# franciscotln/cosmology-model-fit

Hardware: AMD Instinct MI355X
Metric: walker-logL evals/s, Pantheon+ 1701-SN full-cov chi2, theta resident in HBM (higher is better)
Workload: dtype f64; 1 GPU; Pantheon+-shaped 1701-SN full-cov flat-LCDM chi2 + prior, 4096 walkers per GPU per step (BASELINE configs[1] at N=1), G=4000, theta resident in HBM; workload_key=pantheon, walkers_per_gpu=4096, walkers_total=4096, n_sn=1701, n_grid=4000, ndim=4, parallelism=walkers sharded over 1 GPU(s)

## Files before the change

### cosmology-model-fit_amd/_lib.py

```python
from __future__ import annotations

import ctypes as C
import os
import subprocess

_HERE = os.path.dirname(os.path.abspath(__file__))
LIB_PATH = os.environ.get("COSMOFIT_LIB") or os.path.join(_HERE, "libcosmofit_hip.so")
CSRC = os.path.join(_HERE, "csrc")

CF_ABI_VERSION = 11
CF_P_NSLOTS = 15
SLOTS = ("offset", "H0", "Om", "obh2", "och2", "w0", "wa", "v", "rd", "fcc", "lin", "v2", "v3", "s8", "fs8err")

CF_EZ_LATE_FLAT, CF_EZ_PHYSICAL = 0, 1
CF_FDE_LCDM, CF_FDE_WCDM, CF_FDE_THAWING, CF_FDE_CPL = 0, 1, 2, 3
CF_OUT_CHI2, CF_OUT_LOGL, CF_OUT_LOGP = 0, 1, 2
CF_SOLVE_BLOCKED_TRSM, CF_SOLVE_INVERSE_GEMM, CF_SOLVE_AUTO = 0, 1, 2
SOLVE_MODES = {"blocked": CF_SOLVE_BLOCKED_TRSM, "inverse": CF_SOLVE_INVERSE_GEMM, "auto": CF_SOLVE_AUTO}
CF_CMB_NONE = 0
STATUS = {0: "CF_OK", -1: "CF_ERR_INVALID", -2: "CF_ERR_NO_DEVICE", -3: "CF_ERR_HIP", -4: "CF_ERR_NOT_POSDEF",
          -5: "CF_ERR_UNSUPPORTED", -6: "CF_ERR_ILL_CONDITIONED"}


class CosmofitError(RuntimeError):
# ... 200 lines not shown
    "cf_last_kernel_ms": (C.c_int, [_VP, C.POINTER(C.c_float * 2)]),
    "cf_enable_timing": (C.c_int, [_VP, C.c_int]),
    "cf_set_timing_stride": (C.c_int, [_VP, C.c_int]),
    "cf_timed_calls": (C.c_int64, [_VP]),
    "cf_kernel_ms": (C.c_int, [_VP, _I64, C.POINTER(C.c_float * 2)]),
    "cf_kernel_ms3": (C.c_int, [_VP, _I64, C.POINTER(C.c_float * 3)]),
    "cf_walker_form": (C.c_int, [_VP, _I64]),
    "cf_interp_hermite": (C.c_int, [_VP, _I64, _VP, _VP, _VP, _I64, _VP]),
    "cf_interp_pchip": (C.c_int, [_VP, _I64, _VP, _VP, _I64, _VP]),
    "cf_solve_triangular": (C.c_int, [_VP, _I64, _I64, _VP, _I64, _VP]),
    "cf_selftest_invpack_host": (C.c_int, [_VP, _I64, _I64, _VP, C.POINTER(C.c_double), C.POINTER(C.c_double)]),
    "cf_selftest_log10": (C.c_int, [_VP, _I64, _VP]),
    "cf_selftest_log10_tab": (C.c_int, [_VP, _I64, _VP]),
    "cf_selftest_exp_tab": (C.c_int, [_VP, _I64, _VP]),
    "cf_selftest_pos_ops": (C.c_int, [_VP, _VP, _I64, _VP]),
    "cf_ens_active_count": (_I64, [C.c_uint64, _I32, _I32, _I64, _I64]),
    "cf_ens_comp_count": (_I64, [C.c_uint64, _I32, _I32, _I64]),
    "cf_ens_active_set": (C.c_int, [C.c_uint64, _I32, _I32, _I64, _I64, _VP, _VP, _VP]),
    "cf_ens_kde_prepare": (C.c_int, [_VP, _I64, _I32, _I32, _I32, C.c_uint64, _VP, _VP, _VP]),
    "cf_ens_propose": (C.c_int, [_I32, _VP, _I64, _I32, _I32, _I32, C.c_uint64, _VP, _I64, C.c_uint64, C.c_double,
                                 C.c_double, _VP, _VP, _VP, _VP, _VP]),
    "cf_ens_accept": (C.c_int, [_VP, _VP, _I64, C.c_int32, C.c_uint64, _VP, _VP, _VP, _VP, _VP, _VP, _VP]),
    "cf_ens_accept_record": (C.c_int, [_VP, _VP, _I64, C.c_int32, C.c_uint64, _VP, _VP, _VP, _VP, _VP, _VP, _VP, _VP, _VP,
                                       _VP]),
    "cf_chain_mean": (C.c_int, [_VP, _I64, _I64, _VP, _VP]),
    "cf_chain_lagsum": (C.c_int, [_VP, _VP, _I64, _I64, _I64, _I32, _VP, _VP]),
    "cf_chain_acf_mean": (C.c_int, [_VP, _VP, _I64, _I32, _I32, _VP, _VP]),
    "cf_marg_bin": (C.c_int, [_VP, _I64, _I32, _VP, _I32, _VP, _VP]),
    "cf_marg_hist": (C.c_int, [_VP, _VP, C.c_double, _I64, _I32, _I32, _VP, _I32, _VP, _VP, _I32, _VP]),
    "cf_kde_sum_device": (C.c_int, [_VP, _VP, _I64, _I32, _VP, _I64, _I64, _VP, _VP, _VP]),
# ... 98 lines not shown
```

### cosmology-model-fit_amd/csrc/cf_stream_pack.h

```cpp
#ifndef CF_STREAM_PACK_H
#define CF_STREAM_PACK_H

#include <algorithm>
#include <cmath>
#include <cstdint>
#include <numeric>
#include <vector>

#include "cosmofit_device.h"

struct cf_stream_plan {
  std::vector<int32_t> row;
  int32_t seg_off[CF_STREAM_MAX_SEGS + 1];
  int32_t n_seg;
  double max_step, zp1_max;
};

static inline bool cf_stream_assign(const double* z_cmb, const double* step, int64_t n_sn, int n_grid, double inv_step, double z_max,
                                    cf_stream_plan& plan) {
  if (n_grid < 2 || n_grid > CF_STREAM_SEG * CF_STREAM_MAX_SEGS || n_sn < 0 || n_sn > INT32_MAX - CF_STREAM_REC_SLACK) return false;
  plan.n_seg = (n_grid + CF_STREAM_SEG - 1) / CF_STREAM_SEG;
  std::vector<int32_t> node((size_t)n_sn);
  plan.max_step = 0.0;
  plan.zp1_max = 1.0;
// ... 5 lines not shown
  }
  plan.row.resize((size_t)n_sn);
  std::iota(plan.row.begin(), plan.row.end(), 0);
  std::stable_sort(plan.row.begin(), plan.row.end(), [&](int32_t a, int32_t b) { return node[(size_t)a] < node[(size_t)b]; });
  for (int s = 0; s <= CF_STREAM_MAX_SEGS; ++s) plan.seg_off[s] = (int32_t)n_sn;
  int s = 0;
  plan.seg_off[0] = 0;
  for (int64_t j = 0; j < n_sn; ++j) {
    const int sj = cf_stream_segment(node[(size_t)plan.row[(size_t)j]], plan.n_seg);
    while (s < sj) plan.seg_off[++s] = (int32_t)j;
  }
  while (s < CF_STREAM_MAX_SEGS) plan.seg_off[++s] = (int32_t)n_sn;
  return true;
}

#endif
```

### cosmology-model-fit_amd/csrc/cf_wave_scan.h

```cpp
#ifndef CF_WAVE_SCAN_H
#define CF_WAVE_SCAN_H

#include <hip/hip_runtime.h>

template <int CTRL, int ROW_MASK>
__device__ __forceinline__ double dpp_move(double v) {
  const int lo = __builtin_amdgcn_update_dpp(0, __double2loint(v), CTRL, ROW_MASK, 0xF, false);
  const int hi = __builtin_amdgcn_update_dpp(0, __double2hiint(v), CTRL, ROW_MASK, 0xF, false);
  return __hiloint2double(hi, lo);
}

__device__ __forceinline__ double wave_inclusive_scan(double v) {
  v += dpp_move<0x111, 0xF>(v);
  v += dpp_move<0x112, 0xF>(v);
  v += dpp_move<0x114, 0xF>(v);
  v += dpp_move<0x118, 0xF>(v);
  v += dpp_move<0x142, 0xA>(v);
  v += dpp_move<0x143, 0xC>(v);
  return v;
}

#endif
```

### cosmology-model-fit_amd/csrc/cosmofit_api.hip

```cpp
#include <hip/hip_runtime.h>
#include <sys/prctl.h>

#include <cmath>
#include <cstdio>
#include <cstdlib>
#include <chrono>
#include <cstring>
#include <algorithm>
#include <atomic>
#include <utility>
#include <condition_variable>
#include <memory>
#include <mutex>
#include <string>
#include <thread>
#include <vector>

#include "../../include/cosmofit.h"
#include "cf_pack.h"
#include "cf_stream_pack.h"
#include "cosmofit_device.h"
#include "cosmofit_infl.h"
#include "cosmofit_mock.h"
#include "cosmofit_resid.h"
// ... 154 lines not shown
CF_DECLARE_TRIGEMM_SMALL(8, false, 2)
#define CF_DECLARE_TRIGEMM(NP, PF)                                                                                                       \
  extern template __global__ void tri_gemm_chi2_kernel<NP, PF>(const cf_epilogue*, const d2*, int, int, int, const double*, int64_t,     \
                                                               const double*, int64_t, double*, unsigned int*, const double*, double*,  \
                                                               int, unsigned long long*, double*, int, int, int, int, int,              \
                                                               unsigned long long*, unsigned long long);
CF_DECLARE_TRIGEMM(1, 2)
CF_DECLARE_TRIGEMM(2, 2)
extern "C" __global__ void finalize_kernel(cf_epilogue d, const double* theta, int64_t W, const double* chi2_extra,
                                           double* out, int out_kind, unsigned long long* nonfinite, unsigned long long* done_flag,
                                           unsigned long long done_seq);
extern "C" __global__ void interp_kernel(const double* xq, int64_t nq, const double* x, const double* y,
                                         const double* yp, int64_t n, double* out, int mode);
extern "C" __global__ void log10_selftest_kernel(const double* x, int64_t n, double* out, int mode, const cf_d2* tab);
extern "C" __global__ void pos_ops_selftest_kernel(const double* a, const double* b, int64_t n, double* out);
extern "C" __global__ void pad_rhs_kernel(const double* b, int64_t nrhs, int64_t n, int64_t n_ld, double* delta);

static thread_local std::string g_err;

static void default_shape(int& ks, int& tc) {
  ks = 2;
  tc = 4;
}
#define CF_PROBE_LIMIT 1e-11

static int pack_default(const double* L, int64_t n, int64_t ld, cf_host_pack& hp, double* probe_rel = nullptr) {
  int ks, tc;
  default_shape(ks, tc);
  int rc = cf_pack_cholesky(L, n, ld, hp, ks, tc);
  if (rc == 0 && probe_rel) *probe_rel = cf_pack_probe(hp, L, ld);
// ... 127 lines not shown
  InversePack ipack;
  DevBuf partial, arrivals;
  DevBuf partial4;
  DevBuf epi;
  cf_epilogue epi_host{};
  hipStream_t stream = nullptr;
  hipStream_t last_stream = nullptr;
  bool has_last = false;
  std::vector<hipEvent_t> ev;
  int timing_slots = 0, timing_stride = 1;
  int64_t timed_calls = 0, eval_calls = 0;
  cf_dev_desc d{};
  PackedFactor pack;
  DevBuf z_cmb, z_hel, obs, sn_step, sn_rec, log10_tab;
  DevBuf stream_rec, stream_row;
  cf_stream_args sargs{};
  DevBuf bao_z, bao_val, bao_inv_cov, bao_qty, gl_x, gl_w, fixed_mu, cc_z, cc_h, cc_inv_cov, nu_grid, ln_grid, nu_sw, ln_sw, exp2_tab, sn_lin, sn_dir;
  DevBuf theta, out, delta, ypk, chi2_extra, nonfinite;
  DevBuf fs8_z, fs8_val, fs8_inv_cov, fs8_fid, fs8_step_of, fs8_order, fs8_tab, fs8_pts;
  DevBuf bao_nodes, bao_base;
  PinnedBuf done_flags;
  unsigned long long done_seq = 0;
  int done_armed = 0;
  bool theta_on_host = false;
  bool has_small_blocks = false;
  bool has_growth = false;
  cf_qsr_state* qsr = nullptr;
  int64_t max_walkers = 0;
  double pack_probe_rel = 0.0;
  int cu_count = 0;
// ... 410 lines not shown
        rec[i] = cf_d4{d.has_vstep ? 1.0 + c->sn_z_cmb[i] : c->sn_z_cmb[i], d.lin_in_rec ? c->sn_lin_coef[i] : step[i],
                       1.0 + c->sn_z_hel[i], c->sn_obs[i]};
      if (h->sn_rec.ensure(rec.size() * sizeof(cf_d4))) return bail(CF_ERR_HIP);
      if (hipMemcpy(h->sn_rec.p, rec.data(), rec.size() * sizeof(cf_d4), hipMemcpyHostToDevice) != hipSuccess)
        return bail(fail(CF_ERR_HIP, "hipMemcpy(sn_rec) failed"));
      d.sn_rec = h->sn_rec.as<const cf_d4>();
      cf_stream_plan plan;
      if (d.chunk_shift == 3 &&
          cf_stream_assign(c->sn_z_cmb, (d.has_vstep && !d.lin_in_rec) ? step.data() : nullptr, c->n_sn, d.n_grid, d.inv_step, d.z_max, plan)) {
        std::vector<cf_d4> srec((size_t)c->n_sn + CF_STREAM_REC_SLACK, cf_d4{1.0, 1.0, 1.0, 0.0});
        std::vector<int32_t> srow((size_t)c->n_sn + CF_STREAM_REC_SLACK, 0);
        for (int64_t j = 0; j < c->n_sn; ++j) {
          srow[(size_t)j] = plan.row[(size_t)j];
          srec[(size_t)j] = rec[(size_t)plan.row[(size_t)j]];
        }
        int rcs;
        if ((rcs = upload_vec(h->stream_rec, reinterpret_cast<const double*>(srec.data()), (int64_t)srec.size() * 4))) return bail(rcs);
        if (h->stream_row.ensure(srow.size() * sizeof(int32_t))) return bail(CF_ERR_HIP);
        if (hipMemcpy(h->stream_row.p, srow.data(), srow.size() * sizeof(int32_t), hipMemcpyHostToDevice) != hipSuccess)
          return bail(fail(CF_ERR_HIP, "hipMemcpy(stream_row) failed"));
        h->sargs.rec = h->stream_rec.as<const cf_d4>();
        h->sargs.row = h->stream_row.as<const int32_t>();
        for (int s = 0; s <= CF_STREAM_MAX_SEGS; ++s) h->sargs.seg_off[s] = plan.seg_off[s];
        h->sargs.n_seg = plan.n_seg;
        h->sargs.max_step = plan.max_step;
        h->sargs.zp1_max = plan.zp1_max;
      }
      int rc2;
      if ((rc2 = upload_log10_table(h->log10_tab))) return bail(rc2);
      d.log10_tab = h->log10_tab.p;
    }
// ... 1057 lines not shown
    return rc;
  }
  HIP_TRY(hipMemcpy(dx.p, x, (size_t)n * 8, hipMemcpyHostToDevice));
  hipLaunchKernelGGL(log10_selftest_kernel, dim3((unsigned)((n + 255) / 256)), dim3(256), 0, 0, dx.as<const double>(), n,
                     dout.as<double>(), mode, tab.as<const cf_d2>());
  HIP_TRY(hipGetLastError());
  HIP_TRY(hipMemcpy(out, dout.p, (size_t)n * 8, hipMemcpyDeviceToHost));
  return CF_OK;
}
extern "C" int cf_selftest_log10(const double* x, int64_t n, double* out) { return selftest_log10(x, n, out, 0, "cf_selftest_log10"); }
extern "C" int cf_selftest_log10_tab(const double* x, int64_t n, double* out) {
  return selftest_log10(x, n, out, 1, "cf_selftest_log10_tab");
}
extern "C" int cf_selftest_exp_tab(const double* x, int64_t n, double* out) {
  return selftest_log10(x, n, out, 2, "cf_selftest_exp_tab");
}
extern "C" int cf_selftest_pos_ops(const double* a, const double* b, int64_t n, double* out) {
  if (!a || !b || !out || n < 0) return fail(CF_ERR_INVALID, "cf_selftest_pos_ops: bad argument");
  if (cf_device_count() == 0) return fail(CF_ERR_NO_DEVICE, "cf_selftest_pos_ops: no HIP device visible");
  if (n == 0) return CF_OK;
  DevBuf da, db, dout;
  if (da.ensure((size_t)n * 8) || db.ensure((size_t)n * 8) || dout.ensure((size_t)n * 32)) return CF_ERR_HIP;
  HIP_TRY(hipMemcpy(da.p, a, (size_t)n * 8, hipMemcpyHostToDevice));
  HIP_TRY(hipMemcpy(db.p, b, (size_t)n * 8, hipMemcpyHostToDevice));
  hipLaunchKernelGGL(pos_ops_selftest_kernel, dim3((unsigned)((n + 255) / 256)), dim3(256), 0, 0, da.as<const double>(),
                     db.as<const double>(), n, dout.as<double>());
  HIP_TRY(hipGetLastError());
  HIP_TRY(hipMemcpy(out, dout.p, (size_t)n * 32, hipMemcpyDeviceToHost));
  return CF_OK;
}
// ... 1013 lines not shown
```

### cosmology-model-fit_amd/csrc/cosmofit_device.h

```cpp
#ifndef COSMOFIT_DEVICE_H
#define COSMOFIT_DEVICE_H

#include <stdint.h>

#define CF_MAX_NDIM 16
#define CF_MAX_GAUSS 8
#define CF_MAX_BAO 64
#define CF_MAX_GL 256
#define CF_MAX_CC 64
#define CF_MAX_FS8 64
#define CF_N_SLOTS 15

#define CF_BLOCK_TILES 16
#define CF_BLOCK_ROWS 256

#define CF_FDE_LCDM_D 0
#define CF_FDE_WCDM_D 1
#define CF_FDE_THAWING_D 2
#define CF_FDE_CPL_D 3

#define CF_EZ_LATE_FLAT_D 0
#define CF_EZ_PHYSICAL_D 1

#define CF_P_OFFSET_D 0
// ... 105 lines not shown
  const double* nu_sw;
  const double* ln_sw;
  const double* exp2_tab;
  const int32_t* bao_base;
};

#define CF_STREAM_SEG 512
#define CF_STREAM_HALO 64
#define CF_STREAM_WAVES 4
#define CF_STREAM_MAX_SEGS 8
#define CF_STREAM_REC_SLACK 128
#define CF_STREAM_GUARD_NODES (CF_STREAM_HALO / 2 - 4)
struct cf_stream_args {
  const cf_d4* rec;
  const int32_t* row;
  int32_t seg_off[CF_STREAM_MAX_SEGS + 1];
  int32_t n_seg;
  double max_step;
  double zp1_max;
};

#ifdef __HIPCC__
#define CF_HD_INLINE __host__ __device__ static inline
#else
#define CF_HD_INLINE static inline
#endif
CF_HD_INLINE int cf_stream_node(double z, int G, double inv_step, double z_max) {
  if (z <= 0.0) return 0;
  if (!(z < z_max)) return G - 2;
  const int i = (int)(z * inv_step);
// ... 106 lines not shown
```

### cosmology-model-fit_amd/csrc/cosmofit_kernels.hip

```cpp
#include <hip/hip_runtime.h>
#include <type_traits>
#include <stdint.h>

#include "cosmofit_device.h"
#include "cf_wave_scan.h"

typedef double d4 __attribute__((ext_vector_type(4)));
typedef double d2 __attribute__((ext_vector_type(2)));

#define CF_WAVE 64

__device__ __forceinline__ double slot_get(const cf_dev_desc& d, int s, const double* __restrict__ th) {
  const cf_dev_slot& p = d.slot[s];
  return p.idx >= 0 ? p.scale * th[p.idx] : p.fixed;
}

struct ThetaRow {
  double v;
};
__device__ __forceinline__ double readlane_f64(double v, int lane) {
  return __hiloint2double(__builtin_amdgcn_readlane(__double2hiint(v), lane), __builtin_amdgcn_readlane(__double2loint(v), lane));
}
template <class D>
__device__ __forceinline__ double slot_get(const D& d, int s, const ThetaRow& th) {
// ... 291 lines not shown
  const double m = __builtin_amdgcn_frexp_mant(x);
  const d2 t = tab[(__double2hiint(m) >> 14) & 63];
  const double r = fma(m, t.x, -1.0);
  double p = fma_vsv(r, C8, C7);
  p = fma_vvs(p, r, C6);
  p = fma_vvs(p, r, C5);
  p = fma_vvs(p, r, C4);
  p = fma_vvs(p, r, C3);
  p = fma_vvs(p, r, C2);
  p = fma_vvs(p, r, C1);
  const double ek = (double)e;
  return fma_vsv(ek, log10_2hi, t.y) + fma(r, p, ek * log10_2lo);
}


template <int MODEL, int FDE, int CH, bool LAST, class D>
__device__ __forceinline__ double chunk_eval(const D& d, const WalkerCosmo& wc, double c_over_H0, int g0, int lane,
                                             const double (&nu_pre)[CH], const double (&ln)[CH], const double* __restrict__ etab,
                                             double (&dh)[CH], double (&loc)[CH]) {
  const int G = d.n_grid;
  constexpr bool POWER_LAW = FDE == CF_FDE_WCDM_D || FDE == CF_FDE_CPL_D;
  double fde[CH];
  if (POWER_LAW) {
    double x[CH];
#pragma unroll
    for (int k = 0; k < CH; ++k) {
      const int g = g0 + k;
      double z = (double)g * d.step;
      if (LAST) z = g >= G - 1 ? d.z_max : z;
      if (FDE == CF_FDE_CPL_D) {
        const double zp1 = 1.0 + z;
        double r = __builtin_amdgcn_rcp(zp1);
        r = fma(fma(-zp1, r, 1.0), r, r);
        x[k] = fma(3 * (1 + wc.w0 + wc.wa), ln[k], (-3 * wc.wa) * (z * r));
      } else {
// ... 10 lines not shown
      p = fma(p, dx, 1.0 / 120);
      p = fma(p, dx, 1.0 / 24);
      p = fma(p, dx, 1.0 / 6);
      p = fma(p, dx, 0.5);
      p = fma(p * dx, dx, dx);
      fde[k] = fma(fde[k - 1], p, fde[k - 1]);
    }
    if (!(dx_max < 0x1p-5)) {
#pragma unroll
      for (int k = 1; k < CH; ++k) fde[k] = exp_tab(x[k], etab);
    }
  }
#pragma unroll
  for (int k = 0; k < CH; ++k) {
    const int g = g0 + k;
    double z = (double)g * d.step;
    if (LAST) z = g >= G - 1 ? d.z_max : z;
    const double e2 = POWER_LAW ? e2_from_fde<MODEL>(wc, z, fde[k], nu_pre[k]) : e2_of_z<MODEL, FDE, true, D>(d, wc, z, nu_pre[k], ln[k], etab);
    const double v = c_over_H0 * rsqrt_pos(e2);
    dh[k] = (LAST && g >= G) ? 0.0 : v;
  }
  double prev = dpp_move<0x138, 0xF>(dh[CH - 1]);
  double run = 0.0;
  const double half = 0.5 * d.step;
#pragma unroll
  for (int k = 0; k < CH; ++k) {
    const bool counts = (k > 0 || lane > 0) && (!LAST || g0 + k < G);
    run = counts ? fma_vsv(prev + dh[k], half, run) : run;
    loc[k] = run;
    prev = dh[k];
  }
  return run;
}

template <int MODEL, int FDE, int CH, class D>
__device__ __forceinline__ void build_distance_table_regs(const D& d, const WalkerCosmo& wc, d2* tab,
                                                          d4* wave_pub, const double (&nu_pre)[CH], const double (&ln_pre)[CH],
                                                          const double* __restrict__ etab) {
  const int G = d.n_grid;
  const int tid = threadIdx.x, lane = tid & 63, wave = tid >> 6;
  const int g0 = tid * CH;
  const int base = g0 + tid;
  const double c_over_H0 = wc.c / wc.H0;
  double dh[CH], loc[CH];
  const int wave_last = (tid - lane) * CH + 64 * CH - 1;
  const double run = wave_last < G - 1 ? chunk_eval<MODEL, FDE, CH, false>(d, wc, c_over_H0, g0, lane, nu_pre, ln_pre, etab, dh, loc)
                                       : chunk_eval<MODEL, FDE, CH, true>(d, wc, c_over_H0, g0, lane, nu_pre, ln_pre, etab, dh, loc);
  const double incl = wave_inclusive_scan(run);
  const double first_dh = __hiloint2double(__builtin_amdgcn_readfirstlane(__double2hiint(dh[0])),
                                           __builtin_amdgcn_readfirstlane(__double2loint(dh[0])));
  if (lane == 63) wave_pub[wave] = (d4){incl, first_dh, dh[CH - 1], 0.0};
  __syncthreads();
  double term = 0.0;
  if (lane < CF_TPB_A / 64) {
    const d4 pv = wave_pub[lane];
    term = lane < wave ? pv[0] : 0.0;
    if (lane >= 1) {
      const int gb = lane * 64 * CH;
      const double zb = gb == G - 1 ? d.z_max : (double)gb * d.step;
      const double bnd = (wave_pub[lane - 1][2] + pv[1]) / 2 * (zb - (double)(gb - 1) * d.step);
      term += (lane <= wave && gb < G) ? bnd : 0.0;
    }
  }
  term += dpp_move<0x111, 0xF>(term);
  term += dpp_move<0x112, 0xF>(term);
  term += dpp_move<0x114, 0xF>(term);
  const double carry = (incl - run) + __hiloint2double(__builtin_amdgcn_readlane(__double2hiint(term), 7),
                                                       __builtin_amdgcn_readlane(__double2loint(term), 7));
#pragma unroll
  for (int k = 0; k < CH; ++k)
    if (g0 + k < G) tab[base + k] = (d2){loc[k] + carry, dh[k]};
  if (tid > 0 && g0 < G) tab[base - 1] = (d2){loc[0] + carry, dh[0]};
  __syncthreads();
}

template <int MODEL, int FDE>
__device__ __forceinline__ void build_distance_table_lds(const cf_dev_desc& d, const WalkerCosmo& wc, d2* tab,
                                                         d4* wave_pub) {
  double* wave_tot = reinterpret_cast<double*>(wave_pub);
  const int G = d.n_grid, chs = d.chunk_shift, CH = 1 << chs;
  const int tid = threadIdx.x, lane = tid & 63, wave = tid >> 6;
  const int g0 = tid << chs;
  const int base = g0 + tid;
  const int n_own = max(0, min(CH, G - g0));
  const double c_over_H0 = wc.c / wc.H0;
  for (int k = 0; k < n_own; ++k)
    tab[base + k].y = dh_of_node<MODEL, FDE>(d, wc, c_over_H0, g0 + k);
// ... 273 lines not shown
    else sn_fast_loop<false>(d, T, log_tab, out, off, v100, tid, 0.0, part, sn_parts);
  } else if (d.n_sn > 0) {
    double* out = delta + (w >> 4) * (16 * (int64_t)d.n_ld) + 2 * (w & 15);
    if (d.lin_in_rec) sn_fast_loop<false, true, true>(d, T, log_tab, out, off, v100, tid, lin, part, sn_parts);
    else if (d.step_pm1) sn_fast_loop<true, false, true>(d, T, log_tab, out, off, v100, tid, 0.0, part, sn_parts);
    else sn_fast_loop<false, false, true>(d, T, log_tab, out, off, v100, tid, 0.0, part, sn_parts);
  }
}

#define CF_STREAM_WIN ((CF_STREAM_HALO + CF_STREAM_SEG) / 16 * 17)
#define CF_STREAM_Q0 (CF_STREAM_HALO + CF_STREAM_HALO / 16)

__device__ __forceinline__ double uniform_f64(double v) {
  return __hiloint2double(__builtin_amdgcn_readfirstlane(__double2hiint(v)), __builtin_amdgcn_readfirstlane(__double2loint(v)));
}
__device__ __forceinline__ void wave_lds_sync() {
  __builtin_amdgcn_fence(__ATOMIC_RELEASE, "wavefront");
  __builtin_amdgcn_wave_barrier();
  __builtin_amdgcn_fence(__ATOMIC_ACQUIRE, "wavefront");
}

template <bool PM1, bool LIN, bool FAST, class D>
__device__ __forceinline__ void sn_stream_segment(const D& d, const cf_stream_args& sa, const DistTable& T, const d2* __restrict__ log_tab,
                                                  double* __restrict__ out, double off, double v100, double lin, double r_pos,
                                                  double r_neg, double c0, int s, unsigned j, unsigned end, d4 ra, int rowa) {
  auto one_sn = [&](const d4& r, int row) {
    const double za = r[0], st = r[1], zhp1 = r[2], ob = r[3];
    double z_cosmo = za;
    if (!LIN && PM1) {
      z_cosmo = fma(za, st > 0.0 ? r_pos : r_neg, c0);
// ... 30 lines not shown
__global__ void __launch_bounds__(64 * CF_STREAM_WAVES, 4)
walker_stream_kernel(cf_walker_args d, cf_stream_args sa, const double* __restrict__ theta, int64_t W, double* __restrict__ delta,
                     d2* __restrict__ bao_nodes, double* __restrict__ theta_copy) {
  __shared__ __align__(16) d2 win_all[CF_STREAM_WAVES][CF_STREAM_WIN];
  __shared__ __align__(16) d2 log_tab[64];
  __shared__ double exp2_tab[64];

  const int lane = threadIdx.x & 63, wv = __builtin_amdgcn_readfirstlane(threadIdx.x >> 6);
  const int64_t w = (int64_t)blockIdx.x * CF_STREAM_WAVES + wv;
  if (w >= W) return;
  d2* const win = win_all[wv];
  constexpr bool POWER_LAW = FDE == CF_FDE_WCDM_D || FDE == CF_FDE_CPL_D;
  const int G = d.n_grid;
  const ThetaRow th{theta[w * d.ndim + (lane < d.ndim ? lane : 0)]};
  if (theta_copy && lane < d.ndim) theta_copy[w * d.ndim + lane] = th.v;
  log_tab[lane] = reinterpret_cast<const d2*>(d.log10_tab)[lane];
  if (POWER_LAW) exp2_tab[lane] = d.exp2_tab[lane];
  WalkerCosmo wc = make_cosmo(d, th);
  wc.H0 = uniform_f64(wc.H0);
  wc.Om = uniform_f64(wc.Om);
  wc.w0 = uniform_f64(wc.w0);
  wc.wa = uniform_f64(wc.wa);
  wc.Or = uniform_f64(wc.Or);
  wc.Obc = uniform_f64(wc.Obc);
  wc.Ode = uniform_f64(wc.Ode);
  wc.Onu = uniform_f64(wc.Onu);
  const double off = uniform_f64(slot_get(d, CF_P_OFFSET_D, th));
  const double v100 = uniform_f64(100 * slot_get(d, CF_P_V_D, th));
  const double lin = d.lin_in_rec ? uniform_f64(slot_get(d, CF_P_LIN_D, th)) : 0.0;
  const double c_over_H0 = uniform_f64(wc.c / wc.H0);
// ... 4 lines not shown
    r_pos = uniform_f64(1.0 / (1.0 + v100 / d.c));
    r_neg = uniform_f64(1.0 / (1.0 + (-v100) / d.c));
    c0 = -1.0;
  }
  double a_pec;
  const double shift = cf_stream_shift_bound(v100, sa.max_step, sa.zp1_max, d.c, d.inv_step, &a_pec);
  const bool fast = a_pec < 0.5 && shift <= (double)CF_STREAM_GUARD_NODES;
  DistTable T;
  T.G = G;
  T.chs = 4;
  T.step = d.step;
  T.inv_step = d.inv_step;
  T.inv_last = d.inv_last;
  T.z_max = d.z_max;
  double seg_sum = 0.0, seg_bnd = 0.0, prev_last = 0.0;
  wave_lds_sync();
#pragma unroll 1
  for (int s = 0; s < sa.n_seg; ++s) {
    const int g0 = (64 * s + lane) * 8;
    const unsigned sn_j = (unsigned)((fast ? sa.seg_off[s] : 0) + lane), sn_end = (unsigned)(fast ? sa.seg_off[s + 1] : d.n_sn);
    d4 sn_r = (d4){1.0, 1.0, 1.0, 0.0};
    int sn_row = 0;
    if (sn_j < sn_end) {
      sn_r = reinterpret_cast<const d4*>(sa.rec)[sn_j];
      sn_row = sa.row[sn_j];
    }
    double nu_pre[8], ln_pre[8], dh[8], loc[8];
#pragma unroll
    for (int k = 0; k < 8; ++k) {
      nu_pre[k] = MODEL == CF_EZ_PHYSICAL_D ? d.nu_sw[k * CF_TPB_A + 64 * s + lane] : -1.0;
      ln_pre[k] = POWER_LAW ? d.ln_sw[k * CF_TPB_A + 64 * s + lane] : -1.0;
    }
    const int wave_last = CF_STREAM_SEG * s + CF_STREAM_SEG - 1;
    const double run = wave_last < G - 1 ? chunk_eval<MODEL, FDE, 8, false>(d, wc, c_over_H0, g0, lane, nu_pre, ln_pre, exp2_tab, dh, loc)
                                         : chunk_eval<MODEL, FDE, 8, true>(d, wc, c_over_H0, g0, lane, nu_pre, ln_pre, exp2_tab, dh, loc);
    const double incl = wave_inclusive_scan(run);
    const double first_dh = __hiloint2double(__builtin_amdgcn_readfirstlane(__double2hiint(dh[0])),
                                             __builtin_amdgcn_readfirstlane(__double2loint(dh[0])));
    const double tot = readlane_f64(incl, 63), last_dh = readlane_f64(dh[7], 63);
    if (lane == s) {
      seg_sum = tot;
      if (s >= 1) {
        const int gb = s * 64 * 8;
        const double zb = gb == G - 1 ? d.z_max : (double)gb * d.step;
        seg_bnd = (prev_last + first_dh) / 2 * (zb - (double)(gb - 1) * d.step);
      }
    }
    prev_last = last_dh;
    double term = 0.0;
    if (lane < CF_STREAM_MAX_SEGS) {
      term = lane < s ? seg_sum : 0.0;
      if (lane >= 1) term += (lane <= s && lane * 64 * 8 < G) ? seg_bnd : 0.0;
    }
    term += dpp_move<0x111, 0xF>(term);
    term += dpp_move<0x112, 0xF>(term);
    term += dpp_move<0x114, 0xF>(term);
    const double carry = (incl - run) + readlane_f64(term, 7);
    const int base = CF_STREAM_Q0 + 8 * lane + (lane >> 1);
#pragma unroll
    for (int k = 0; k < 8; ++k)
      if (g0 + k < G) win[base + k] = (d2){loc[k] + carry, dh[k]};
    if (!(lane & 1) && g0 < G) win[base - 1] = (d2){loc[0] + carry, dh[0]};
    wave_lds_sync();
    T.tab = win + (CF_STREAM_Q0 - (CF_STREAM_SEG / 16 * 17) * s);
    for (int e = lane; e < CF_BAO_NODES * d.n_aux; e += 64) {
      const int k = e / CF_BAO_NODES, o = e % CF_BAO_NODES;
      const int g = d.bao_base[k] + o;
      if (min(g / CF_STREAM_SEG, sa.n_seg - 1) == s) bao_nodes[(w * d.n_aux + k) * CF_BAO_NODES + o] = T.at(g);
    }
#define CF_STREAM_SN(PM1, LIN, LINV, RP, RN, C0)                                                                                  \
  (fast ? sn_stream_segment<PM1, LIN, true>(d, sa, T, log_tab, out, off, v100, LINV, RP, RN, C0, s, sn_j, sn_end, sn_r, sn_row)  \
        : sn_stream_segment<PM1, LIN, false>(d, sa, T, log_tab, out, off, v100, LINV, RP, RN, C0, s, sn_j, sn_end, sn_r, sn_row))
    if (d.lin_in_rec) CF_STREAM_SN(false, true, lin, 1.0, 1.0, 0.0);
    else if (d.step_pm1) CF_STREAM_SN(true, false, 0.0, r_pos, r_neg, c0);
    else CF_STREAM_SN(false, false, 0.0, 1.0, 1.0, 0.0);
#undef CF_STREAM_SN
    if (s + 1 < sa.n_seg) {
// ... 1354 lines not shown
  const double t2 = t * t, t3 = t2 * t;
  const double h00 = 2 * t3 - 3 * t2 + 1, h10 = t3 - 2 * t2 + t, h01 = -2 * t3 + 3 * t2, h11 = t3 - t2;
  out[k] = h00 * y[i] + h10 * h_i * d_i + h01 * y[i + 1] + h11 * h_i * d_i1;
}

extern "C" __global__ void pos_ops_selftest_kernel(const double* __restrict__ a, const double* __restrict__ b, int64_t n,
                                                   double* __restrict__ out) {
  const int64_t k = blockIdx.x * (int64_t)blockDim.x + threadIdx.x;
  if (k >= n) return;
  out[4 * k + 0] = sqrt_pos(a[k]);
  out[4 * k + 1] = sqrt(a[k]);
  out[4 * k + 2] = div_pos(a[k], b[k]);
  out[4 * k + 3] = a[k] / b[k];
}

extern "C" __global__ void log10_selftest_kernel(const double* __restrict__ x, int64_t n, double* __restrict__ out, int mode,
                                                 const cf_d2* __restrict__ tab) {
  const int64_t k = blockIdx.x * (int64_t)blockDim.x + threadIdx.x;
  if (k >= n) return;
  if (mode == 2) out[k] = exp_tab(x[k], reinterpret_cast<const double*>(tab));
  else out[k] = mode == 0 ? log10_pos(x[k]) : log10_tab(x[k], reinterpret_cast<const d2*>(tab));
}

extern "C" __global__ void pad_rhs_kernel(const double* __restrict__ b, int64_t nrhs, int64_t n, int64_t n_ld,
                                          double* __restrict__ delta) {
  const int64_t w = blockIdx.x;
  for (int64_t i = threadIdx.x; i < n_ld; i += blockDim.x) delta[w * n_ld + i] = (w < nrhs && i < n) ? b[w * n + i] : 0.0;
}
```

### include/cosmofit.h

```cpp
#ifndef COSMOFIT_H
#define COSMOFIT_H

#include <stdint.h>

#ifdef __cplusplus
extern "C" {
#endif

#define CF_ABI_VERSION 11

typedef struct cf_handle cf_handle;

enum cf_status {
  CF_OK = 0,
  CF_ERR_INVALID = -1,
  CF_ERR_NO_DEVICE = -2,
  CF_ERR_HIP = -3,
  CF_ERR_NOT_POSDEF = -4,
  CF_ERR_UNSUPPORTED = -5,
  CF_ERR_ILL_CONDITIONED = -6
};

enum cf_ez_model {
  CF_EZ_LATE_FLAT = 0,
// ... 221 lines not shown
int cf_interp_pchip(const double* xq, int64_t nq, const double* x, const double* y, int64_t n,
                    double* out);
int cf_solve_triangular(const double* L, int64_t n, int64_t ld, const double* b, int64_t nrhs,
                        double* out);

int cf_selftest_pack_host(const double* L, int64_t n, int64_t ld, const double* b, double* chi2_out,
                          int64_t* packed_bytes);

int cf_selftest_invpack_host(const double* L, int64_t n, int64_t ld, const double* b, double* chi2_out,
                             double* probe_out);

int cf_selftest_log10(const double* x, int64_t n, double* out);
int cf_selftest_log10_tab(const double* x, int64_t n, double* out);
int cf_selftest_exp_tab(const double* x, int64_t n, double* out);
int cf_selftest_pos_ops(const double* a, const double* b, int64_t n, double* out);

int64_t cf_ens_active_count(uint64_t split_key, int32_t n_splits, int32_t split, int64_t shard_start, int64_t shard_stop);
int64_t cf_ens_comp_count(uint64_t split_key, int32_t n_splits, int32_t split, int64_t w_total);
int cf_ens_active_set(uint64_t split_key, int32_t n_splits, int32_t split, int64_t shard_start, int64_t shard_stop,
                      int64_t* d_ids, int64_t* d_local_idx, void* hip_stream);
int cf_ens_kde_prepare(const double* d_all_pos, int64_t w_total, int32_t ndim, int32_t n_splits, int32_t split,
                       uint64_t split_key, double* d_params, double* d_wc, void* hip_stream);
int cf_ens_propose(int32_t kind, const double* d_all_pos, int64_t w_total, int32_t ndim, int32_t n_splits, int32_t split,
                   uint64_t split_key, const int64_t* d_ids, int64_t n_active, uint64_t key0, double a, double de_sigma,
                   const double* d_kde_params, const double* d_kde_wc, double* d_y, double* d_log_factor,
                   void* hip_stream);
int cf_ens_accept(const int64_t* d_ids, const int64_t* d_local_idx, int64_t n_active, int32_t ndim, uint64_t key0,
                  const double* d_y, const double* d_lp_new, const double* d_log_factor, double* d_x_local,
                  double* d_logp_local, uint64_t* d_n_accepted, void* hip_stream);
int cf_ens_accept_record(const int64_t* d_ids, const int64_t* d_local_idx, int64_t n_active, int32_t ndim, uint64_t key0,
// ... 313 lines not shown
```

Before: 18.46 million evals/s.

## Tabulate (1+z)^3 for flat LCDM streaming kernel, prefetch per segment, trim DPP and stores

For flat LambdaCDM the streaming walker kernel now reads a precomputed (1+z)^3 grid table from HBM. The table for the next segment is prefetched while the current one is integrated, so E^2 becomes a single FMA instead of the general e2_of_z path. It also sets bound_ctrl on the row-shift DPP moves and drops the per-element bounds checks on stores for inner segments. The cost is extra memory traffic and registers per segment, plus explicit waitcnt and asm barriers that could stall or limit occupancy.

```diff
diff --git a/cosmology-model-fit_amd/_lib.py b/cosmology-model-fit_amd/_lib.py
--- a/cosmology-model-fit_amd/_lib.py
+++ b/cosmology-model-fit_amd/_lib.py
@@ -238,6 +238,7 @@
     "cf_selftest_log10_tab": (C.c_int, [_VP, _I64, _VP]),
     "cf_selftest_exp_tab": (C.c_int, [_VP, _I64, _VP]),
     "cf_selftest_pos_ops": (C.c_int, [_VP, _VP, _I64, _VP]),
+    "cf_selftest_zp3": (C.c_int, [C.c_int32, C.c_double, _VP, _VP, _I64]),
     "cf_ens_active_count": (_I64, [C.c_uint64, _I32, _I32, _I64, _I64]),
     "cf_ens_comp_count": (_I64, [C.c_uint64, _I32, _I32, _I64]),
     "cf_ens_active_set": (C.c_int, [C.c_uint64, _I32, _I32, _I64, _I64, _VP, _VP, _VP]),
diff --git a/cosmology-model-fit_amd/csrc/cf_stream_pack.h b/cosmology-model-fit_amd/csrc/cf_stream_pack.h
--- a/cosmology-model-fit_amd/csrc/cf_stream_pack.h
+++ b/cosmology-model-fit_amd/csrc/cf_stream_pack.h
@@ -43,4 +43,18 @@
   return true;
 }
 
+static inline bool cf_stream_zp3_table(int n_grid, double step, double z_max, std::vector<double>& zp3) {
+  if (n_grid < 2 || n_grid > CF_STREAM_SEG * CF_STREAM_MAX_SEGS) return false;
+  const int n_seg = (n_grid + CF_STREAM_SEG - 1) / CF_STREAM_SEG;
+  zp3.assign((size_t)CF_STREAM_SEG * (size_t)n_seg, 1.0);
+  for (int g = 0; g < n_grid; ++g) {
+    double z = (double)g * step;
+    if (g == n_grid - 1) z = z_max;
+    const double zp1 = 1.0 + z;
+    const double sq = zp1 * zp1;
+    zp3[(size_t)g] = sq * zp1;
+  }
+  return true;
+}
+
 #endif
diff --git a/cosmology-model-fit_amd/csrc/cf_wave_scan.h b/cosmology-model-fit_amd/csrc/cf_wave_scan.h
--- a/cosmology-model-fit_amd/csrc/cf_wave_scan.h
+++ b/cosmology-model-fit_amd/csrc/cf_wave_scan.h
@@ -3,18 +3,20 @@
 
 #include <hip/hip_runtime.h>
 
-template <int CTRL, int ROW_MASK>
+template <int CTRL, int ROW_MASK, bool BC = false>
 __device__ __forceinline__ double dpp_move(double v) {
-  const int lo = __builtin_amdgcn_update_dpp(0, __double2loint(v), CTRL, ROW_MASK, 0xF, false);
-  const int hi = __builtin_amdgcn_update_dpp(0, __double2hiint(v), CTRL, ROW_MASK, 0xF, false);
+  static_assert(!BC || ROW_MASK == 0xF, "bound_ctrl gives the zero only to lanes of enabled rows");
+  const int lo = __builtin_amdgcn_update_dpp(0, __double2loint(v), CTRL, ROW_MASK, 0xF, BC);
+  const int hi = __builtin_amdgcn_update_dpp(0, __double2hiint(v), CTRL, ROW_MASK, 0xF, BC);
   return __hiloint2double(hi, lo);
 }
 
+template <bool BC = false>
 __device__ __forceinline__ double wave_inclusive_scan(double v) {
-  v += dpp_move<0x111, 0xF>(v);
-  v += dpp_move<0x112, 0xF>(v);
-  v += dpp_move<0x114, 0xF>(v);
-  v += dpp_move<0x118, 0xF>(v);
+  v += dpp_move<0x111, 0xF, BC>(v);
+  v += dpp_move<0x112, 0xF, BC>(v);
+  v += dpp_move<0x114, 0xF, BC>(v);
+  v += dpp_move<0x118, 0xF, BC>(v);
   v += dpp_move<0x142, 0xA>(v);
   v += dpp_move<0x143, 0xC>(v);
   return v;
diff --git a/cosmology-model-fit_amd/csrc/cosmofit_api.hip b/cosmology-model-fit_amd/csrc/cosmofit_api.hip
--- a/cosmology-model-fit_amd/csrc/cosmofit_api.hip
+++ b/cosmology-model-fit_amd/csrc/cosmofit_api.hip
@@ -192,6 +192,7 @@
                                          const double* yp, int64_t n, double* out, int mode);
 extern "C" __global__ void log10_selftest_kernel(const double* x, int64_t n, double* out, int mode, const cf_d2* tab);
 extern "C" __global__ void pos_ops_selftest_kernel(const double* a, const double* b, int64_t n, double* out);
+extern "C" __global__ void zp3_selftest_kernel(int n_grid, double step, double z_max, double* out);
 extern "C" __global__ void pad_rhs_kernel(const double* b, int64_t nrhs, int64_t n, int64_t n_ld, double* delta);
 
 static thread_local std::string g_err;
@@ -349,6 +350,7 @@
   PackedFactor pack;
   DevBuf z_cmb, z_hel, obs, sn_step, sn_rec, log10_tab;
   DevBuf stream_rec, stream_row;
+  DevBuf stream_zp3;
   cf_stream_args sargs{};
   DevBuf bao_z, bao_val, bao_inv_cov, bao_qty, gl_x, gl_w, fixed_mu, cc_z, cc_h, cc_inv_cov, nu_grid, ln_grid, nu_sw, ln_sw, exp2_tab, sn_lin, sn_dir;
   DevBuf theta, out, delta, ypk, chi2_extra, nonfinite;
@@ -789,7 +791,11 @@
           srow[(size_t)j] = plan.row[(size_t)j];
           srec[(size_t)j] = rec[(size_t)plan.row[(size_t)j]];
         }
+        std::vector<double> zp3;
+        if (!cf_stream_zp3_table(d.n_grid, d.step, d.z_max, zp3)) return bail(fail(CF_ERR_INVALID, "cf_create: internal: no (1 + z)^3 table"));
         int rcs;
+        if ((rcs = upload_vec(h->stream_zp3, zp3.data(), (int64_t)zp3.size()))) return bail(rcs);
+        h->sargs.zp3 = h->stream_zp3.as<const double>();
         if ((rcs = upload_vec(h->stream_rec, reinterpret_cast<const double*>(srec.data()), (int64_t)srec.size() * 4))) return bail(rcs);
         if (h->stream_row.ensure(srow.size() * sizeof(int32_t))) return bail(CF_ERR_HIP);
         if (hipMemcpy(h->stream_row.p, srow.data(), srow.size() * sizeof(int32_t), hipMemcpyHostToDevice) != hipSuccess)
@@ -1877,6 +1883,21 @@
 }
 extern "C" int cf_selftest_exp_tab(const double* x, int64_t n, double* out) {
   return selftest_log10(x, n, out, 2, "cf_selftest_exp_tab");
+}
+extern "C" int cf_selftest_zp3(int32_t n_grid, double z_max, double* device_cube, double* host_table, int64_t n) {
+  if (!device_cube || !host_table || n_grid < 2) return fail(CF_ERR_INVALID, "cf_selftest_zp3: bad argument");
+  if (cf_device_count() == 0) return fail(CF_ERR_NO_DEVICE, "cf_selftest_zp3: no HIP device visible");
+  const double step = z_max / (double)(n_grid - 1);
+  std::vector<double> zp3;
+  if (!cf_stream_zp3_table(n_grid, step, z_max, zp3)) return fail(CF_ERR_UNSUPPORTED, "cf_selftest_zp3: the grid does not fit the streaming kernel");
+  if (n != (int64_t)zp3.size()) return fail(CF_ERR_INVALID, "cf_selftest_zp3: n must be 512 * ceil(n_grid / 512)");
+  std::copy(zp3.begin(), zp3.end(), host_table);
+  DevBuf dout;
+  if (dout.ensure((size_t)n * 8)) return CF_ERR_HIP;
+  hipLaunchKernelGGL(zp3_selftest_kernel, dim3((unsigned)(n / 512)), dim3(64), 0, 0, n_grid, step, z_max, dout.as<double>());
+  HIP_TRY(hipGetLastError());
+  HIP_TRY(hipMemcpy(device_cube, dout.p, (size_t)n * 8, hipMemcpyDeviceToHost));
+  return CF_OK;
 }
 extern "C" int cf_selftest_pos_ops(const double* a, const double* b, int64_t n, double* out) {
   if (!a || !b || !out || n < 0) return fail(CF_ERR_INVALID, "cf_selftest_pos_ops: bad argument");
diff --git a/cosmology-model-fit_amd/csrc/cosmofit_device.h b/cosmology-model-fit_amd/csrc/cosmofit_device.h
--- a/cosmology-model-fit_amd/csrc/cosmofit_device.h
+++ b/cosmology-model-fit_amd/csrc/cosmofit_device.h
@@ -143,6 +143,7 @@
 struct cf_stream_args {
   const cf_d4* rec;
   const int32_t* row;
+  const double* zp3;
   int32_t seg_off[CF_STREAM_MAX_SEGS + 1];
   int32_t n_seg;
   double max_step;
diff --git a/cosmology-model-fit_amd/csrc/cosmofit_kernels.hip b/cosmology-model-fit_amd/csrc/cosmofit_kernels.hip
--- a/cosmology-model-fit_amd/csrc/cosmofit_kernels.hip
+++ b/cosmology-model-fit_amd/csrc/cosmofit_kernels.hip
@@ -329,11 +329,26 @@
 }
 
 
-template <int MODEL, int FDE, int CH, bool LAST, class D>
-__device__ __forceinline__ double chunk_eval(const D& d, const WalkerCosmo& wc, double c_over_H0, int g0, int lane,
-                                             const double (&nu_pre)[CH], const double (&ln)[CH], const double* __restrict__ etab,
-                                             double (&dh)[CH], double (&loc)[CH]) {
-  const int G = d.n_grid;
+#ifndef CF_WB_TABLE
+#define CF_WB_TABLE 1
+#endif
+#ifndef CF_WB_STORES
+#define CF_WB_STORES 1
+#endif
+#ifndef CF_WB_DPP
+#define CF_WB_DPP 1
+#endif
+constexpr bool kWbDpp = CF_WB_DPP != 0;
+
+template <int MODEL, int FDE, int CH, bool LAST, bool ZP3, class D>
+__device__ __forceinline__ double chunk_eval_zp3(const D& d, const WalkerCosmo& wc, double c_over_H0, int g0, int lane,
+                                                 const double (&nu_pre)[CH], const double (&ln)[CH], const double* __restrict__ etab,
+                                                 const double (&zp3)[CH], double (&dh)[CH], double (&loc)[CH]) {
+  static_assert(!ZP3 || (MODEL == CF_EZ_LATE_FLAT_D && FDE == CF_FDE_LCDM_D), "only flat LambdaCDM takes the tabulated cubes");
+  int G = d.n_grid;
+#if CF_WB_STORES
+  if (LAST) asm volatile("" : "+s"(G));
+#endif
   constexpr bool POWER_LAW = FDE == CF_FDE_WCDM_D || FDE == CF_FDE_CPL_D;
   double fde[CH];
   if (POWER_LAW) {
@@ -374,13 +389,18 @@
 #pragma unroll
   for (int k = 0; k < CH; ++k) {
     const int g = g0 + k;
-    double z = (double)g * d.step;
-    if (LAST) z = g >= G - 1 ? d.z_max : z;
-    const double e2 = POWER_LAW ? e2_from_fde<MODEL>(wc, z, fde[k], nu_pre[k]) : e2_of_z<MODEL, FDE, true, D>(d, wc, z, nu_pre[k], ln[k], etab);
+    double e2;
+    if constexpr (ZP3) {
+      e2 = wc.Om * zp3[k] + (1.0 - wc.Om);
+    } else {
+      double z = (double)g * d.step;
+      if (LAST) z = g >= G - 1 ? d.z_max : z;
+      e2 = POWER_LAW ? e2_from_fde<MODEL>(wc, z, fde[k], nu_pre[k]) : e2_of_z<MODEL, FDE, true, D>(d, wc, z, nu_pre[k], ln[k], etab);
+    }
     const double v = c_over_H0 * rsqrt_pos(e2);
     dh[k] = (LAST && g >= G) ? 0.0 : v;
   }
-  double prev = dpp_move<0x138, 0xF>(dh[CH - 1]);
+  double prev = dpp_move<0x138, 0xF, kWbDpp>(dh[CH - 1]);
   double run = 0.0;
   const double half = 0.5 * d.step;
 #pragma unroll
@@ -391,6 +411,12 @@
     prev = dh[k];
   }
   return run;
+}
+template <int MODEL, int FDE, int CH, bool LAST, class D>
+__device__ __forceinline__ double chunk_eval(const D& d, const WalkerCosmo& wc, double c_over_H0, int g0, int lane,
+                                             const double (&nu_pre)[CH], const double (&ln)[CH], const double* __restrict__ etab,
+                                             double (&dh)[CH], double (&loc)[CH]) {
+  return chunk_eval_zp3<MODEL, FDE, CH, LAST, false>(d, wc, c_over_H0, g0, lane, nu_pre, ln, etab, nu_pre, dh, loc);
 }
 
 template <int MODEL, int FDE, int CH, class D>
@@ -404,9 +430,10 @@
   const double c_over_H0 = wc.c / wc.H0;
   double dh[CH], loc[CH];
   const int wave_last = (tid - lane) * CH + 64 * CH - 1;
-  const double run = wave_last < G - 1 ? chunk_eval<MODEL, FDE, CH, false>(d, wc, c_over_H0, g0, lane, nu_pre, ln_pre, etab, dh, loc)
-                                       : chunk_eval<MODEL, FDE, CH, true>(d, wc, c_over_H0, g0, lane, nu_pre, ln_pre, etab, dh, loc);
-  const double incl = wave_inclusive_scan(run);
+  const bool inner = wave_last < G - 1;
+  const double run = inner ? chunk_eval<MODEL, FDE, CH, false>(d, wc, c_over_H0, g0, lane, nu_pre, ln_pre, etab, dh, loc)
+                           : chunk_eval<MODEL, FDE, CH, true>(d, wc, c_over_H0, g0, lane, nu_pre, ln_pre, etab, dh, loc);
+  const double incl = wave_inclusive_scan<kWbDpp>(run);
   const double first_dh = __hiloint2double(__builtin_amdgcn_readfirstlane(__double2hiint(dh[0])),
                                            __builtin_amdgcn_readfirstlane(__double2loint(dh[0])));
   if (lane == 63) wave_pub[wave] = (d4){incl, first_dh, dh[CH - 1], 0.0};
@@ -422,15 +449,21 @@
       term += (lane <= wave && gb < G) ? bnd : 0.0;
     }
   }
-  term += dpp_move<0x111, 0xF>(term);
-  term += dpp_move<0x112, 0xF>(term);
-  term += dpp_move<0x114, 0xF>(term);
+  term += dpp_move<0x111, 0xF, kWbDpp>(term);
+  term += dpp_move<0x112, 0xF, kWbDpp>(term);
+  term += dpp_move<0x114, 0xF, kWbDpp>(term);
   const double carry = (incl - run) + __hiloint2double(__builtin_amdgcn_readlane(__double2hiint(term), 7),
                                                        __builtin_amdgcn_readlane(__double2loint(term), 7));
-#pragma unroll
-  for (int k = 0; k < CH; ++k)
-    if (g0 + k < G) tab[base + k] = (d2){loc[k] + carry, dh[k]};
-  if (tid > 0 && g0 < G) tab[base - 1] = (d2){loc[0] + carry, dh[0]};
+  if (CF_WB_STORES && inner) {
+#pragma unroll
+    for (int k = 0; k < CH; ++k) tab[base + k] = (d2){loc[k] + carry, dh[k]};
+    if (tid > 0) tab[base - 1] = (d2){loc[0] + carry, dh[0]};
+  } else {
+#pragma unroll
+    for (int k = 0; k < CH; ++k)
+      if (g0 + k < G) tab[base + k] = (d2){loc[k] + carry, dh[k]};
+    if (tid > 0 && g0 < G) tab[base - 1] = (d2){loc[0] + carry, dh[0]};
+  }
   __syncthreads();
 }
 
@@ -734,6 +767,7 @@
 __device__ __forceinline__ double uniform_f64(double v) {
   return __hiloint2double(__builtin_amdgcn_readfirstlane(__double2hiint(v)), __builtin_amdgcn_readfirstlane(__double2loint(v)));
 }
+__device__ __forceinline__ void stream_landed(double& v) { asm volatile("" : "+v"(v)); }
 __device__ __forceinline__ void wave_lds_sync() {
   __builtin_amdgcn_fence(__ATOMIC_RELEASE, "wavefront");
   __builtin_amdgcn_wave_barrier();
@@ -794,6 +828,18 @@
   const int G = d.n_grid;
   const ThetaRow th{theta[w * d.ndim + (lane < d.ndim ? lane : 0)]};
   if (theta_copy && lane < d.ndim) theta_copy[w * d.ndim + lane] = th.v;
+  constexpr bool ZP3 = CF_WB_TABLE && MODEL == CF_EZ_LATE_FLAT_D && FDE == CF_FDE_LCDM_D;
+  double zp3[8] = {};
+  auto fetch_zp3 = [&](int seg) {
+    const d2* __restrict__ src = reinterpret_cast<const d2*>(sa.zp3) + (unsigned)((64 * seg + lane) * 4);
+#pragma unroll
+    for (int k = 0; k < 4; ++k) {
+      const d2 v = src[k];
+      zp3[2 * k] = v.x;
+      zp3[2 * k + 1] = v.y;
+    }
+  };
+  if (ZP3) fetch_zp3(0);
   log_tab[lane] = reinterpret_cast<const d2*>(d.log10_tab)[lane];
   if (POWER_LAW) exp2_tab[lane] = d.exp2_tab[lane];
   WalkerCosmo wc = make_cosmo(d, th);
@@ -828,10 +874,15 @@
   T.inv_last = d.inv_last;
   T.z_max = d.z_max;
   double seg_sum = 0.0, seg_bnd = 0.0, prev_last = 0.0;
+  if (ZP3) {
+#pragma unroll
+    for (int k = 0; k < 8; ++k) stream_landed(zp3[k]);
+  }
   wave_lds_sync();
 #pragma unroll 1
   for (int s = 0; s < sa.n_seg; ++s) {
     const int g0 = (64 * s + lane) * 8;
+    if (ZP3) __builtin_amdgcn_s_waitcnt(0x0F70);
     const unsigned sn_j = (unsigned)((fast ? sa.seg_off[s] : 0) + lane), sn_end = (unsigned)(fast ? sa.seg_off[s + 1] : d.n_sn);
     d4 sn_r = (d4){1.0, 1.0, 1.0, 0.0};
     int sn_row = 0;
@@ -846,9 +897,12 @@
       ln_pre[k] = POWER_LAW ? d.ln_sw[k * CF_TPB_A + 64 * s + lane] : -1.0;
     }
     const int wave_last = CF_STREAM_SEG * s + CF_STREAM_SEG - 1;
-    const double run = wave_last < G - 1 ? chunk_eval<MODEL, FDE, 8, false>(d, wc, c_over_H0, g0, lane, nu_pre, ln_pre, exp2_tab, dh, loc)
-                                         : chunk_eval<MODEL, FDE, 8, true>(d, wc, c_over_H0, g0, lane, nu_pre, ln_pre, exp2_tab, dh, loc);
-    const double incl = wave_inclusive_scan(run);
+    const bool inner = wave_last < G - 1;
+    const double run =
+        inner ? chunk_eval_zp3<MODEL, FDE, 8, false, ZP3>(d, wc, c_over_H0, g0, lane, nu_pre, ln_pre, exp2_tab, zp3, dh, loc)
+              : chunk_eval_zp3<MODEL, FDE, 8, true, ZP3>(d, wc, c_over_H0, g0, lane, nu_pre, ln_pre, exp2_tab, zp3, dh, loc);
+    if (ZP3 && s + 1 < sa.n_seg) fetch_zp3(s + 1);
+    const double incl = wave_inclusive_scan<kWbDpp>(run);
     const double first_dh = __hiloint2double(__builtin_amdgcn_readfirstlane(__double2hiint(dh[0])),
                                              __builtin_amdgcn_readfirstlane(__double2loint(dh[0])));
     const double tot = readlane_f64(incl, 63), last_dh = readlane_f64(dh[7], 63);
@@ -866,15 +920,25 @@
       term = lane < s ? seg_sum : 0.0;
       if (lane >= 1) term += (lane <= s && lane * 64 * 8 < G) ? seg_bnd : 0.0;
     }
-    term += dpp_move<0x111, 0xF>(term);
-    term += dpp_move<0x112, 0xF>(term);
-    term += dpp_move<0x114, 0xF>(term);
+    term += dpp_move<0x111, 0xF, kWbDpp>(term);
+    term += dpp_move<0x112, 0xF, kWbDpp>(term);
+    term += dpp_move<0x114, 0xF, kWbDpp>(term);
     const double carry = (incl - run) + readlane_f64(term, 7);
     const int base = CF_STREAM_Q0 + 8 * lane + (lane >> 1);
-#pragma unroll
-    for (int k = 0; k < 8; ++k)
-      if (g0 + k < G) win[base + k] = (d2){loc[k] + carry, dh[k]};
-    if (!(lane & 1) && g0 < G) win[base - 1] = (d2){loc[0] + carry, dh[0]};
+    if (CF_WB_STORES && inner) {
+#pragma unroll
+      for (int k = 0; k < 8; ++k) win[base + k] = (d2){loc[k] + carry, dh[k]};
+      if (!(lane & 1)) win[base - 1] = (d2){loc[0] + carry, dh[0]};
+    } else {
+#pragma unroll
+      for (int k = 0; k < 8; ++k)
+        if (g0 + k < G) win[base + k] = (d2){loc[k] + carry, dh[k]};
+      if (!(lane & 1) && g0 < G) win[base - 1] = (d2){loc[0] + carry, dh[0]};
+    }
+    if (ZP3) {
+#pragma unroll
+      for (int k = 0; k < 8; ++k) stream_landed(zp3[k]);
+    }
     wave_lds_sync();
     T.tab = win + (CF_STREAM_Q0 - (CF_STREAM_SEG / 16 * 17) * s);
     for (int e = lane; e < CF_BAO_NODES * d.n_aux; e += 64) {
@@ -2259,6 +2323,21 @@
   out[4 * k + 3] = a[k] / b[k];
 }
 
+extern "C" __global__ void zp3_selftest_kernel(int n_grid, double step, double z_max, double* __restrict__ out) {
+  const int G = n_grid, s = blockIdx.x, lane = threadIdx.x;
+  const int g0 = (64 * s + lane) * 8;
+  const bool last = !(CF_STREAM_SEG * s + CF_STREAM_SEG - 1 < G - 1);
+#pragma unroll
+  for (int k = 0; k < 8; ++k) {
+    const int g = g0 + k;
+    double z = (double)g * step;
+    if (last) z = g >= G - 1 ? z_max : z;
+    const double zp1 = 1.0 + z;
+    const double cubed = zp1 * zp1 * zp1;
+    out[g] = g < G ? cubed : 1.0;
+  }
+}
+
 extern "C" __global__ void log10_selftest_kernel(const double* __restrict__ x, int64_t n, double* __restrict__ out, int mode,
                                                  const cf_d2* __restrict__ tab) {
   const int64_t k = blockIdx.x * (int64_t)blockDim.x + threadIdx.x;
diff --git a/include/cosmofit.h b/include/cosmofit.h
--- a/include/cosmofit.h
+++ b/include/cosmofit.h
@@ -259,6 +259,7 @@
 int cf_selftest_log10_tab(const double* x, int64_t n, double* out);
 int cf_selftest_exp_tab(const double* x, int64_t n, double* out);
 int cf_selftest_pos_ops(const double* a, const double* b, int64_t n, double* out);
+int cf_selftest_zp3(int32_t n_grid, double z_max, double* device_cube, double* host_table, int64_t n);
 
 int64_t cf_ens_active_count(uint64_t split_key, int32_t n_splits, int32_t split, int64_t shard_start, int64_t shard_stop);
 int64_t cf_ens_comp_count(uint64_t split_key, int32_t n_splits, int32_t split, int64_t w_total);
```

Result: no change. 18.55 million evals/s, median of 6 (+0.5%).
